# Kmatsuo57/cell-image-analysis

Hardware: AMD Instinct MI355X
Metric: cells/sec screened (CAE fwd + recon-MSE + SVM score), 64x64 (higher is better)
Workload: dtype f32 (results in the fp32 error class; the contractions run as split 16-bit products on the matrix pipe, fp32 accumulate: conv1..conv6 as 2 fp16 terms x 3 products with exact power-of-two scales from each cell's own data, the PCA GEMM as 3 bf16 terms x 6 products, conv7's 32 -> 16 channel contraction; 1 GPU; BASELINE.json configs[2]: screening inference, 1000000 synthetic 64x64 crops on one GPU, resident in HBM, CAE fwd + recon MSE/MAE + RobustScaler + PCA(100) + 2x OCSVM score on device; cells_per_gpu=1000000, global_cells=1000000, chunk_cells=65536, detector_train_cells=5000, weights=random init (Glorot, non-trivial BN), seed 42, parallelism=dp1

## Files before the change

cell-image-analysis_amd/csrc/conv12_fused.hip:

```cpp
#include "kernel_setup.hpp"
#include "split16.hpp"

#include <cmath>
#include <cstdlib>
#include <cstring>
#include <type_traits>
#include <vector>

namespace cs {

namespace {

constexpr int NTHR = 512;
constexpr int V_BYTES = 36 * 2048;
constexpr int RING_SLOTS = 10;
constexpr int RING_ROWF = 34 * 32 + 8;
static_assert((4 * RING_ROWF) % 64 == 32 && RING_ROWF % 2 == 0, "ring pitch");
constexpr int RING_BYTES = RING_SLOTS * RING_ROWF * 4;
constexpr int E2_BYTES = 8 * 2048;
constexpr int INP_STRIDE = 72;
constexpr int INP_BYTES = 67 * INP_STRIDE * 4;
constexpr int OFF_RING = V_BYTES;
constexpr int OFF_E2 = OFF_RING + RING_BYTES;
constexpr int OFF_INP = OFF_E2 + E2_BYTES;
// ... 116 lines not shown
    if (tid < 384) ((float*)(smem + OFF_B1))[tid] = w1frag[tid];
    if (tid < 32) {
        const float sc = ep1[32 + tid];
        ((f32x4*)(smem + OFF_EP1))[tid] = f32x4{ep1[tid], sc, ep1[64 + tid], sc >= 0.0f ? 1.0f : -1.0f};
    }
    if (tid >= 64 && tid < 128) {
        const int c = tid - 64;
        const float sc = ep2[64 + c];
        ((f32x4*)(smem + OFF_EP2))[c] = f32x4{ep2[c], sc, ep2[128 + c], sc >= 0.0f ? 1.0f : -1.0f};
    }
    if constexpr (C1H) {
        for (int i = tid; i < (2 * 2 * 64 * 16) / 4; i += NTHR) ((unsigned int*)(smem + OFF_B1X))[i] = w1x3[i];
    }
    {
        const int srow = tid >> 4, sc16 = tid & 15;
        const float* src = x + (size_t)blockIdx.x * 4096 + srow * 64 + 4 * sc16;
        float* dst = inp + (srow + 1) * INP_STRIDE + 4 + 4 * sc16;
        f32x4 c0 = *(const f32x4*)src, c1 = *(const f32x4*)(src + 32 * 64);
        c12_sanitize(c0);
        c12_sanitize(c1);
        *(f32x4*)dst = c0;
        *(f32x4*)(dst + 32 * INP_STRIDE) = c1;
        if constexpr (C2H) {
            const unsigned int mx = f16x2_rowmax(f16x2_absmax8(c0, c1));
            if ((lane & 15) == 0) atomicMax((unsigned int*)(smem + OFF_XMAX), mx);
        }
    }
    __syncthreads();
    float vscale = 1.0f, vunscale = 1.0f, xscale = 1.0f, xunscale = 1.0f;
    auto set_scale = [&]() {
        const float xm = __builtin_bit_cast(float, *(const unsigned int*)(smem + OFF_XMAX));
        if constexpr (C1H) {
            int Ex = (int)((__builtin_bit_cast(unsigned int, xm) >> 23) & 0xffu);
            Ex = Ex < 40 ? 40 : (Ex > 254 ? 254 : Ex);
            Ex = __builtin_amdgcn_readfirstlane(Ex);
            xscale = __builtin_bit_cast(float, (unsigned int)(268 - Ex) << 23);
            xunscale = __builtin_bit_cast(float, (unsigned int)(Ex - 14) << 23) * inv_sw1;
        }
        const float vb = 100.0f * fmaf(p1a, xm, p1b);
        int E = (int)((__builtin_bit_cast(unsigned int, vb) >> 23) & 0xffu);
        E = E < 40 ? 40 : (E > 254 ? 254 : E);
        E = __builtin_amdgcn_readfirstlane(E);
        vscale = __builtin_bit_cast(float, (unsigned int)(268 - E) << 23);
        vunscale = __builtin_bit_cast(float, (unsigned int)(E - 14) << 23) * inv_sw;
    };
    if constexpr (C2H) set_scale();
    auto records_in_place = [&](int t) {
        float* p0 = inp + ((t >> 4) + 1) * INP_STRIDE + 4 + 4 * (t & 15);
// ... 152 lines not shown
                const float* const rcol = ring + (4 * tx) * 32 + 2 * p;
                auto p2_body = [&](auto lo_c) {
                    constexpr bool LO = decltype(lo_c)::value;
                    f32x2 t[3][6];
                    {
                        const float* rrow[5];
    #pragma unroll
                        for (int m = 0; m < 5; ++m) {
                            const unsigned int sm = (unsigned int)(rbase + m);
                            const unsigned int slot = min(sm, sm - (unsigned int)RING_SLOTS);
                            rrow[m] = rcol + slot * RING_ROWF;
                        }
                        f32x2 d[6][5];
    #pragma unroll
                        for (int j = 0; j < 6; ++j)
    #pragma unroll
                            for (int m = 0; m < 5; ++m) d[j][m] = lds_read_b64(rrow[m] + j * 32);
                        if (g == 3 && has_next) {
                            float* dst = inp + ((t2 >> 4) + 1) * INP_STRIDE + 4 + 4 * (t2 & 15);
                            c12_sanitize(stg0);
                            c12_sanitize(stg1);
                            *(f32x4*)dst = stg0;
                            *(f32x4*)(dst + 32 * INP_STRIDE) = stg1;
                            const unsigned int mx = f16x2_rowmax(f16x2_absmax8(stg0, stg1));
                            if ((l2 & 15) == 0) atomicMax((unsigned int*)(smem + OFF_XMAX), mx);
                        }
    #pragma unroll
                        for (int j = 0; j < 6; ++j) {
                            f32x2 o[3];
                            bt6_half<LO>(d[j], o);
    #pragma unroll
                            for (int rr = 0; rr < 3; ++rr) t[rr][j] = o[rr];
                        }
                    }
                    const int sx = (tile >> 1) & 7;
                    char* const vhi = smem + (3 * h) * (6 * 2048) + (tile * 8 + ((p >> 2) ^ sx)) * 16 + (p & 3) * 4;
                    char* const vlo = smem + (3 * h) * (6 * 2048) + (tile * 8 + ((4 + (p >> 2)) ^ sx)) * 16 + (p & 3) * 4;
    #pragma unroll
                    for (int rr = 0; rr < 3; ++rr) {
                        f32x2 o[6];
                        bt6_pair(t[rr], o);
                        unsigned int ph[6], pl[6];
                        f16x2_split6_pairs(o, ph, pl);
    #pragma unroll
                        for (int c = 0; c < 6; ++c) {
                            *(unsigned int*)(vhi + (rr * 6 + c) * 2048) = ph[c];
                            *(unsigned int*)(vlo + (rr * 6 + c) * 2048) = pl[c];
                        }
// ... 316 lines not shown
```

cell-image-analysis_amd/csrc/conv45_h2.hip:

```cpp
#include "kernel_setup.hpp"
#include "split16.hpp"

#include <cstring>

namespace cs {

namespace {

constexpr int G = 8;
constexpr int CH = 32;
constexpr int WP = G + 2;
constexpr int PXB = 64;
constexpr int ROWB = WP * PXB + 32;
constexpr int PLANE = WP * ROWB;
constexpr int WG_PER_CU = 2;

constexpr int C5_OUT = 64;

constexpr int H2_OFF_MAX = 2 * PLANE;
constexpr int H2_LDS_BYTES = 2 * PLANE + 16;

__device__ __forceinline__ void h2_split_store(char* dst, const f32x4& x, float S)
{
    f16x4 hi;
// ... 15 lines not shown
    const int th = wave >> 1;
    const int li = lane & 15, kq = lane >> 4;

    f16x8 B[9][2];
#pragma unroll
    for (int t = 0; t < 9; ++t)
#pragma unroll
        for (int p = 0; p < 2; ++p) B[t][p] = wfrag[((slice * 9 + t) * 2 + p) * 64 + lane];
    const int co = slice * 16 + li;
    const float bias = ep[co], bns = ep[CH + co], bnt = ep[2 * CH + co];

    for (int i = tid; i < H2_LDS_BYTES / 16; i += 256) *(f32x4*)(smem + i * 16) = f32x4{0.0f, 0.0f, 0.0f, 0.0f};

    long cell = blockIdx.x;
    if (cell >= n_cells) return;
    f32x4 stg[2];
#pragma unroll
    for (int k = 0; k < 2; ++k) stg[k] = *(const f32x4*)(in + (size_t)cell * (G * G * CH) + (tid + 256 * k) * 4);
    __syncthreads();
    {
        unsigned int mx = 0;
        f16x2_absmax4(stg[0], mx);
        f16x2_absmax4(stg[1], mx);
        mx = f16x2_rowmax(mx);
        if (li == 0) atomicMax(&mxw[0], mx);
    }
    __syncthreads();
    float S, invS;
    f16x2_scale(mxw[0], S, invS);

    int woff[2];
#pragma unroll
    for (int k = 0; k < 2; ++k) {
        const int idx = tid + 256 * k, px = idx >> 3, c4 = idx & 7;
        woff[k] = ((px >> 3) + 1) * ROWB + ((px & 7) + 1) * PXB + c4 * 8;
    }
    const int abase = (4 * th + (li >> 3)) * ROWB + (li & 7) * PXB + kq * 16;

    for (int it = 0; cell < n_cells; cell += gridDim.x, ++it) {
        const float unscale = invS * inv_sw;
#pragma unroll
        for (int k = 0; k < 2; ++k) h2_split_store(smem + woff[k], stg[k], S);
        __syncthreads();
        if (tid == 0) mxw[it & 1] = 0;
        const long ncell = cell + gridDim.x;
        if (ncell < n_cells) {
#pragma unroll
            for (int k = 0; k < 2; ++k) stg[k] = *(const f32x4*)(in + (size_t)ncell * (G * G * CH) + (tid + 256 * k) * 4);
// ... 7 lines not shown
#pragma unroll
            for (int t = 0; t < 2; ++t) {
                const char* a = smem + abase + toff + t * (2 * ROWB);
                const f16x8 a1 = *(const f16x8*)a;
                const f16x8 a2 = *(const f16x8*)(a + PLANE);
                lo[t] = __builtin_amdgcn_mfma_f32_16x16x32_f16(a1, B[tap][1], lo[t], 0, 0, 0);
                hi[t] = __builtin_amdgcn_mfma_f32_16x16x32_f16(a1, B[tap][0], hi[t], 0, 0, 0);
                lo[t] = __builtin_amdgcn_mfma_f32_16x16x32_f16(a2, B[tap][0], lo[t], 0, 0, 0);
            }
        }
#pragma unroll
        for (int t = 0; t < 2; ++t) {
            float* o = out + ((size_t)cell * (G * G) + 16 * (2 * th + t) + 4 * kq) * CH + co;
#pragma unroll
            for (int r = 0; r < 4; ++r) {
                const float v = fmaxf(fmaf(hi[t][r] + lo[t][r], unscale, bias), 0.0f);
                o[r * CH] = fmaf(v, bns, bnt);
            }
        }
        if (ncell < n_cells) {
            unsigned int mx = 0;
            f16x2_absmax4(stg[0], mx);
            f16x2_absmax4(stg[1], mx);
            mx = f16x2_rowmax(mx);
            if (li == 0) atomicMax(&mxw[(it + 1) & 1], mx);
        }
        __syncthreads();
        f16x2_scale(mxw[(it + 1) & 1], S, invS);
    }
}

__global__ __launch_bounds__(512, 2) void conv5_h2_kernel(const float* __restrict__ in, const f16x8* __restrict__ wfrag,
                                                          const float* __restrict__ ep, float* __restrict__ out, long n_cells, float inv_sw)
{
    extern __shared__ __attribute__((aligned(16))) char smem[];
    unsigned int* const mxw = (unsigned int*)(smem + H2_OFF_MAX);
    const int tid = threadIdx.x;
    const int lane = tid & 63;
    const int wave = __builtin_amdgcn_readfirstlane(tid >> 6);
    const int ph = wave >> 1, pa = ph >> 1, pb = ph & 1;
    const int sp = wave & 1;
    const int li = lane & 15, kq = lane >> 4;

    f16x8 B[4][2][2];
#pragma unroll
    for (int t = 0; t < 4; ++t)
#pragma unroll
        for (int k = 0; k < 2; ++k)
#pragma unroll
            for (int p = 0; p < 2; ++p) B[t][k][p] = wfrag[(((wave * 4 + t) * 2 + k) * 2 + p) * 64 + lane];
    float bias[2], bns[2], bnt[2];
#pragma unroll
    for (int k = 0; k < 2; ++k) {
        const int co = (2 * sp + k) * 16 + li;
        bias[k] = ep[co]; bns[k] = ep[C5_OUT + co]; bnt[k] = ep[2 * C5_OUT + co];
    }

    for (int i = tid; i < H2_LDS_BYTES / 16; i += 512) *(f32x4*)(smem + i * 16) = f32x4{0.0f, 0.0f, 0.0f, 0.0f};

    long cell = blockIdx.x;
    if (cell >= n_cells) return;
    f32x4 stg = *(const f32x4*)(in + (size_t)cell * (G * G * CH) + tid * 4);
    __syncthreads();
    {
        unsigned int mx = 0;
        f16x2_absmax4(stg, mx);
        mx = f16x2_rowmax(mx);
        if (li == 0) atomicMax(&mxw[0], mx);
    }
    __syncthreads();
    float S, invS;
    f16x2_scale(mxw[0], S, invS);
    const int woff = ((tid >> 6) + 1) * ROWB + (((tid >> 3) & 7) + 1) * PXB + (tid & 7) * 8;
    const int abase = ((li >> 3) + pa) * ROWB + ((li & 7) + pb) * PXB + kq * 16;

    for (int it = 0; cell < n_cells; cell += gridDim.x, ++it) {
        const float unscale = invS * inv_sw;
        h2_split_store(smem + woff, stg, S);
        __syncthreads();
        if (tid == 0) mxw[it & 1] = 0;
        const long ncell = cell + gridDim.x;
        if (ncell < n_cells) stg = *(const f32x4*)(in + (size_t)ncell * (G * G * CH) + tid * 4);

        float* obase = out + (((size_t)cell * (2 * G) + pa) * (2 * G) + pb) * C5_OUT + (2 * sp) * 16 + li;
#pragma unroll
        for (int t = 0; t < 4; ++t) {
            f32x4 ah[2] = {{0.0f, 0.0f, 0.0f, 0.0f}, {0.0f, 0.0f, 0.0f, 0.0f}};
            f32x4 al[2] = {{0.0f, 0.0f, 0.0f, 0.0f}, {0.0f, 0.0f, 0.0f, 0.0f}};
#pragma unroll
            for (int tap = 0; tap < 4; ++tap) {
                const char* a = smem + abase + t * (2 * ROWB) + (tap >> 1) * ROWB + (tap & 1) * PXB;
                const f16x8 a1 = *(const f16x8*)a;
                const f16x8 a2 = *(const f16x8*)(a + PLANE);
#pragma unroll
                for (int k = 0; k < 2; ++k) {
                    al[k] = __builtin_amdgcn_mfma_f32_16x16x32_f16(a1, B[tap][k][1], al[k], 0, 0, 0);
                    ah[k] = __builtin_amdgcn_mfma_f32_16x16x32_f16(a1, B[tap][k][0], ah[k], 0, 0, 0);
                    al[k] = __builtin_amdgcn_mfma_f32_16x16x32_f16(a2, B[tap][k][0], al[k], 0, 0, 0);
                }
            }
#pragma unroll
            for (int r = 0; r < 4; ++r) {
                const int i = 4 * kq + r, ys = 2 * t + (i >> 3), xs = i & 7;
                float* o = obase + ((size_t)(2 * ys) * (2 * G) + 2 * xs) * C5_OUT;
#pragma unroll
                for (int k = 0; k < 2; ++k) {
                    const float v = fmaxf(fmaf(ah[k][r] + al[k][r], unscale, bias[k]), 0.0f);
                    o[16 * k] = fmaf(v, bns[k], bnt[k]);
                }
            }
        }
        if (ncell < n_cells) {
            unsigned int mx = 0;
            f16x2_absmax4(stg, mx);
            mx = f16x2_rowmax(mx);
            if (li == 0) atomicMax(&mxw[(it + 1) & 1], mx);
        }
        __syncthreads();
        f16x2_scale(mxw[(it + 1) & 1], S, invS);
    }
}

constexpr int F45_OFF_A = 2 * PLANE;
constexpr int F45_OFF_W4 = 4 * PLANE;
constexpr int F45_W4_BYTES = 2 * 9 * 2 * 64 * 16;
constexpr int F45_OFF_MAX = F45_OFF_W4 + F45_W4_BYTES;
constexpr int F45_LDS_BYTES = F45_OFF_MAX + 16;
static_assert(2 * F45_LDS_BYTES <= 160 * 1024, "two workgroups per CU");

__global__ __launch_bounds__(512, 2) void conv45_h2_kernel(const float* __restrict__ in , const f16x8* __restrict__ w4frag,
                                                           const float* __restrict__ ep4, float inv_sw4, const f16x8* __restrict__ w5frag,
                                                           const float* __restrict__ ep5, float inv_sw5, float* __restrict__ out ,
                                                           long n_cells)
{
    extern __shared__ __attribute__((aligned(16))) char smem[];
    unsigned int* const mxw = (unsigned int*)(smem + F45_OFF_MAX);
    const int tid = threadIdx.x;
    const int lane = tid & 63;
    const int wave = __builtin_amdgcn_readfirstlane(tid >> 6);
// ... 8 lines not shown
#pragma unroll
        for (int k = 0; k < 2; ++k)
#pragma unroll
            for (int p = 0; p < 2; ++p) B[t][k][p] = w5frag[(((wave * 4 + t) * 2 + k) * 2 + p) * 64 + lane];
    float bias[2], bns[2], bnt[2];
#pragma unroll
    for (int k = 0; k < 2; ++k) {
        const int co = (2 * sp + k) * 16 + li;
        bias[k] = ep5[co]; bns[k] = ep5[C5_OUT + co]; bnt[k] = ep5[2 * C5_OUT + co];
    }
    const int co4 = slice4 * 16 + li;
    const float bias4 = ep4[co4], bns4 = ep4[CH + co4], bnt4 = ep4[2 * CH + co4];

    for (int i = tid; i < F45_LDS_BYTES / 16; i += 512) *(f32x4*)(smem + i * 16) = f32x4{0.0f, 0.0f, 0.0f, 0.0f};
    __syncthreads();
    for (int i = tid; i < F45_W4_BYTES / 16; i += 512) *(f16x8*)(smem + F45_OFF_W4 + i * 16) = w4frag[i];

    long cell = blockIdx.x;
    if (cell >= n_cells) return;
    f32x4 stg = *(const f32x4*)(in + (size_t)cell * (G * G * CH) + tid * 4);
    {
        unsigned int mx = 0;
        f16x2_absmax4(stg, mx);
        mx = f16x2_rowmax(mx);
        if (li == 0) atomicMax(&mxw[0], mx);
    }
    __syncthreads();
    float S3, invS3;
    f16x2_scale(mxw[0], S3, invS3);
    const int woff = ((tid >> 6) + 1) * ROWB + (((tid >> 3) & 7) + 1) * PXB + (tid & 7) * 8;
    const int abase4 = (2 * tile4 + (li >> 3)) * ROWB + (li & 7) * PXB + kq * 16;
    const char* const w4l = smem + F45_OFF_W4 + (size_t)slice4 * 9 * 2 * 64 * 16 + lane * 16;
    const int abase5 = F45_OFF_A + ((li >> 3) + pa) * ROWB + ((li & 7) + pb) * PXB + kq * 16;

    for (int it = 0; cell < n_cells; cell += gridDim.x, ++it) {
        h2_split_store(smem + woff, stg, S3);
        __syncthreads();
        if (tid == 0) mxw[it & 1] = 0;
        const long ncell = cell + gridDim.x;
        if (ncell < n_cells) stg = *(const f32x4*)(in + (size_t)ncell * (G * G * CH) + tid * 4);

        f32x4 a4v;
        {
            f32x4 hi = {0.0f, 0.0f, 0.0f, 0.0f}, lo = {0.0f, 0.0f, 0.0f, 0.0f};
#pragma unroll
            for (int tap = 0; tap < 9; ++tap) {
                const char* a = smem + abase4 + (tap / 3) * ROWB + (tap % 3) * PXB;
                const f16x8 a1 = *(const f16x8*)a;
                const f16x8 a2 = *(const f16x8*)(a + PLANE);
                const f16x8 bh = *(const f16x8*)(w4l + (tap * 2 + 0) * 1024), bl = *(const f16x8*)(w4l + (tap * 2 + 1) * 1024);
                lo = __builtin_amdgcn_mfma_f32_16x16x32_f16(a1, bl, lo, 0, 0, 0);
                hi = __builtin_amdgcn_mfma_f32_16x16x32_f16(a1, bh, hi, 0, 0, 0);
                lo = __builtin_amdgcn_mfma_f32_16x16x32_f16(a2, bh, lo, 0, 0, 0);
            }
            const float us4 = invS3 * inv_sw4;
            float am = 0.0f;
#pragma unroll
            for (int r = 0; r < 4; ++r) {
                const float v = fmaxf(fmaf(hi[r] + lo[r], us4, bias4), 0.0f);
                a4v[r] = fmaf(v, bns4, bnt4);
                am = fmaxf(am, fabsf(a4v[r]));
            }
            const unsigned int m = f16x2_rowmax(__builtin_bit_cast(unsigned int, am));
            if (li == 0) atomicMax(&mxw[2 + (it & 1)], m);
        }
        __syncthreads();
        float S4, invS4;
        f16x2_scale(mxw[2 + (it & 1)], S4, invS4);
        {
#pragma unroll
            for (int r = 0; r < 4; ++r) {
                const int p = 16 * tile4 + 4 * kq + r;
                char* d = smem + F45_OFF_A + ((p >> 3) + 1) * ROWB + ((p & 7) + 1) * PXB + co4 * 2;
                const float v = a4v[r] * S4;
                const _Float16 h = (_Float16)v;
                *(_Float16*)d = h;
                *(_Float16*)(d + PLANE) = (_Float16)(v - (float)h);
            }
        }
        __syncthreads();
        if (tid == 0) mxw[2 + (it & 1)] = 0;

        const float unscale = invS4 * inv_sw5;
        float* obase = out + (((size_t)cell * (2 * G) + pa) * (2 * G) + pb) * C5_OUT + (2 * sp) * 16 + li;
#pragma unroll
        for (int t = 0; t < 4; ++t) {
            f32x4 ah[2] = {{0.0f, 0.0f, 0.0f, 0.0f}, {0.0f, 0.0f, 0.0f, 0.0f}};
// ... 4 lines not shown
                const f16x8 a1 = *(const f16x8*)a;
                const f16x8 a2 = *(const f16x8*)(a + PLANE);
#pragma unroll
                for (int k = 0; k < 2; ++k) {
                    al[k] = __builtin_amdgcn_mfma_f32_16x16x32_f16(a1, B[tap][k][1], al[k], 0, 0, 0);
                    ah[k] = __builtin_amdgcn_mfma_f32_16x16x32_f16(a1, B[tap][k][0], ah[k], 0, 0, 0);
                    al[k] = __builtin_amdgcn_mfma_f32_16x16x32_f16(a2, B[tap][k][0], al[k], 0, 0, 0);
                }
            }
#pragma unroll
            for (int r = 0; r < 4; ++r) {
                const int i = 4 * kq + r, ys = 2 * t + (i >> 3), xs = i & 7;
                float* o = obase + ((size_t)(2 * ys) * (2 * G) + 2 * xs) * C5_OUT;
#pragma unroll
                for (int k = 0; k < 2; ++k) {
                    const float v = fmaxf(fmaf(ah[k][r] + al[k][r], unscale, bias[k]), 0.0f);
                    o[16 * k] = fmaf(v, bns[k], bnt[k]);
                }
            }
        }
        if (ncell < n_cells) {
            unsigned int mx = 0;
            f16x2_absmax4(stg, mx);
            mx = f16x2_rowmax(mx);
            if (li == 0) atomicMax(&mxw[(it + 1) & 1], mx);
        }
        __syncthreads();
        f16x2_scale(mxw[(it + 1) & 1], S3, invS3);
    }
}

}

size_t pack_conv4_f16x2(const float* hwio, uint16_t* dst, float* inv_sw)
{
    const size_t n = (size_t)2 * 9 * 2 * 64 * 8;
    if (!dst) return n;
    const float S = f16x2_weight_scale(hwio, (size_t)9 * CH * CH);
    if (inv_sw) *inv_sw = 1.0f / S;
    for (int s = 0; s < 2; ++s)
        for (int t = 0; t < 9; ++t)
            for (int l = 0; l < 64; ++l)
                for (int j = 0; j < 8; ++j) {
                    const int li = l & 15, kq = l >> 4;
                    uint16_t pl[2];
                    f16x2_split(hwio[((size_t)t * CH + 8 * kq + j) * CH + 16 * s + li], S, pl[0], pl[1]);
                    for (int p = 0; p < 2; ++p) dst[((((size_t)s * 9 + t) * 2 + p) * 64 + l) * 8 + j] = pl[p];
                }
// ... 58 lines not shown
```

cell-image-analysis_amd/csrc/conv_wino_cs.hip:

```cpp
#include "kernel_setup.hpp"
#include "split16.hpp"

#include <cmath>
#include <cstdlib>
#include <cstring>
#include <vector>

namespace cs {

namespace {

template <int H_, int W_, int CIN_, int COUT_>
struct WinoCfg {
    static constexpr int H = H_, W = W_, CIN = CIN_, COUT = COUT_;
    static constexpr int TW = W / 2;
    static constexpr int TR = 16 / TW;
    static constexpr int SR = 2 * TR;
    static constexpr int R = SR + 2, WP = W + 2;
    static constexpr int PS = CIN + 4;
    static constexpr int STRIP = R * WP * PS * 4;
    static constexpr int NQ = CIN / 16, NS = COUT / 16, KS = CIN / 4;
    static constexpr int NB = 4 * NS * KS;
    static constexpr int XCH = 4 * NS * 2 * 64 * 16;
    static constexpr int LDS = 2 * STRIP + XCH;
// ... 240 lines not shown

    const long total = n_cells * C::NGRP;
    const long first = blockIdx.x;
    if (first >= total) return;
    const int spx = tid / C::C4, sc4 = tid % C::C4;
    const int goff = spx * C::CIN + sc4 * 4, loff = (spx + 1) * C::PS + sc4 * 4;
    auto cell_ptr = [&](long cell) { return in + (size_t)cell * C::H * C::W * C::CIN; };
    auto st_prep = [&](int y0, int r, f32x4 v, unsigned int& mx) {
        const int sy = y0 - 1 + r;
        if (sy < 0 || sy >= C::H) v = f32x4{0.0f, 0.0f, 0.0f, 0.0f};
        f16x2_absmax4(v, mx);
        return v;
    };
    for (int i = tid; i < W3H::LDS / 16; i += 256) ((f32x4*)smem)[i] = f32x4{0.0f, 0.0f, 0.0f, 0.0f};
    __syncthreads();
    float S, invS;
    {
        unsigned int mx = 0;
#pragma unroll
        for (int r = 0; r < C::R; ++r) {
            const f32x4 v = st_prep((int)(first % C::NGRP) * C::SR, r, wn_load<C>(cell_ptr(first / C::NGRP), (int)(first % C::NGRP) * C::SR, r, goff), mx);
            *(f32x4*)((float*)smem + r * W3X::ROWP + loff) = v;
        }
        mx = f16x2_rowmax(mx);
        if (li == 0) atomicMax(&mxw[0], mx);
        __syncthreads();
        f16x2_scale<2>(mxw[0], S, invS);
        __syncthreads();
        if (tid == 0) mxw[0] = 0;
    }

    f32x4 stg[C::NLD];
    int buf = 0;
    int k = 0;
    for (long item = first; item < total; item += gridDim.x, ++k) {
        const long cell = item / C::NGRP;
        const int grp = (int)(item % C::NGRP);
        const long nitem = item + gridDim.x;
        const bool has_next = nitem < total;
        const float* strip = (const float*)(smem + buf * W3X::STRIP);
        float* nstrip = (float*)(smem + (buf ^ 1) * W3X::STRIP);
        unsigned int* const mword = mxw + ((k + 1) & 1);
        const float unscale = invS * inv_sw;
        if (has_next) {
#pragma unroll
            for (int j = 0; j < C::NLD; ++j) stg[j] = wn_load<C>(cell_ptr(nitem / C::NGRP), (int)(nitem % C::NGRP) * C::SR, j, goff);
        }
        const float* da_p = strip + poff + ca * C::PS;
// ... 30 lines not shown
                    acc[s][r] = d;
                }
            }
        }
#pragma unroll
        for (int s = 0; s < C::NS; ++s) {
            f32x4 s0, s1;
#pragma unroll
            for (int r = 0; r < 4; ++r) {
                s0[r] = (acc[s][0][r] + acc[s][1][r]) + acc[s][2][r];
                s1[r] = (acc[s][1][r] - acc[s][2][r]) - acc[s][3][r];
            }
            float* x = xch + ((size_t)((wc * C::NS + s) * 2) * 64 + lane) * 4;
            *(f32x4*)x = s0;
            *(f32x4*)(x + 64 * 4) = s1;
        }
        if (has_next) {
            unsigned int mx = 0;
#pragma unroll
            for (int j = 0; j < C::NLD; ++j) {
                stg[j] = st_prep((int)(nitem % C::NGRP) * C::SR, j, stg[j], mx);
                *(f32x4*)(nstrip + j * W3X::ROWP + loff) = stg[j];
            }
            mx = f16x2_rowmax(mx);
            if (li == 0) atomicMax(mword, mx);
        }
        __syncthreads();
        if (has_next) f16x2_scale<2>(*mword, S, invS);
        f32x4 t0[4], t1[4];
#pragma unroll
        for (int c = 0; c < 4; ++c) {
            const float* x = xch + ((size_t)((c * C::NS + fs) * 2) * 64 + lane) * 4;
            t0[c] = *(const f32x4*)x;
            t1[c] = *(const f32x4*)(x + 64 * 4);
        }
        const f32x4 y00 = (t0[0] + t0[1]) + t0[2], y01 = (t0[1] - t0[2]) - t0[3];
        const f32x4 y10 = (t1[0] + t1[1]) + t1[2], y11 = (t1[1] - t1[2]) - t1[3];
        auto post = [&](float v) { v = fmaxf(fmaf(v, unscale, bias), 0.0f); return fmaf(v, bns, bnt); };
#pragma unroll
        for (int rr = 0; rr < C::FR; ++rr) {
            const float a = rbase ? y00[2 + rr] : y00[rr], b = rbase ? y01[2 + rr] : y01[rr];
            const float c2 = rbase ? y10[2 + rr] : y10[rr], d = rbase ? y11[2 + rr] : y11[rr];
            const float mx = fmaxf(fmaxf(a, b), fmaxf(c2, d)), mn = fminf(fminf(a, b), fminf(c2, d));
            const float res = post(bns >= 0.0f ? mx : mn);
            const int t = 4 * kq + rbase + rr;
            const int ty = grp * C::TR + t / C::TW, tx = t % C::TW;
            out[(((size_t)cell * (C::H / 2) + ty) * (C::W / 2) + tx) * C::COUT + co] = res;
        }
// ... 284 lines not shown
```

cell-image-analysis_amd/csrc/conv_wino_up.hip:

```cpp
#include "kernel_setup.hpp"
#include "split16.hpp"

#include <type_traits>

#include <cmath>
#include <cstdlib>
#include <cstring>

namespace cs {

namespace {

template <int HS_, int WS_, int CIN_, int COUT_>
struct WUCfg {
    static constexpr int HS = HS_, WS = WS_, CIN = CIN_, COUT = COUT_;
    static constexpr int HO = 2 * HS, WO = 2 * WS;
    static constexpr int TW = WS / 2;
    static constexpr int SR = 2 * (16 / TW);
    static constexpr int R = SR + 2, WP = WS + 2;
    static constexpr int PS = CIN + 4;
    static constexpr int STRIP = R * WP * PS * 4;
    static constexpr int LDS = 2 * STRIP;
    static constexpr int NGRP = HS / SR;
    static constexpr int NQ = CIN / 16, KS = CIN / 4;
// ... 454 lines not shown
#pragma unroll
            for (int p = 0; p < 2; ++p) B[t][k][p] = wfrag[(((wave * 4 + t) * 2 + k) * 2 + p) * 64 + lane];
    const int co = wsl * 16 + li;
    const int cosw = co ^ ((kq & 1) << 4);
    const float bias = ep[co], bns = ep[C::COUT + co], bnt = ep[2 * C::COUT + co];
    const float b7 = b7p[0];

    const long first = blockIdx.x;
    if (first >= n_cells) return;
    const int se = tid & (C::EPR - 1), rsub = tid / C::EPR;
    const int spx = se / C::C4, sc4 = se & (C::C4 - 1);
    const int goff = spx * C::CIN + sc4 * 4;
    const int loffb = (spx + 1) * F67H::PXB + sc4 * 8;
    auto cell_ptr = [&](long cell) { return in + (size_t)cell * C::HS * C::WS * C::CIN; };
    for (int i = tid; i < F67H::LDS / 16; i += C::THREADS) ((f32x4*)smem)[i] = f32x4{0.0f, 0.0f, 0.0f, 0.0f};
    __syncthreads();
    wl[(tid >> 5) * F67H::WP + (tid & 31)] = weff[tid];
    float unscale;
    {
        f32x4 stg[C::NLD];
        unsigned int mx = 0;
#pragma unroll
        for (int j = 0; j < C::NLD; ++j) stg[j] = h2_prep(0, j, rsub, wu_load<C>(cell_ptr(first), 0, j, rsub, goff), mx);
        mx = f16x2_rowmax(mx);
        if (li == 0) atomicMax(&mxw[0], mx);
        __syncthreads();
        float S, invS;
        f16x2_scale(mxw[0], S, invS);
        unscale = invS * inv_sw;
#pragma unroll
        for (int j = 0; j < C::NLD; ++j) h2_store(smem, j, rsub, loffb, stg[j], S);
    }
    __syncthreads();
    if (tid == 0) mxw[0] = 0;
    const char* abase = smem + (pa * 18 + li + pb) * F67H::PXB + kq * 16;

    int strip_no = 0;
    for (long cell = first; cell < n_cells; cell += gridDim.x) {
        const float* xc = x + (size_t)cell * 64 * 64;
        float s2 = 0.0f, s1 = 0.0f;
#pragma unroll 1
        for (int grp = 0; grp < C::NGRP; ++grp) {
            const long ncell = grp < C::NGRP - 1 ? cell : cell + gridDim.x;
            const int ngrp = grp < C::NGRP - 1 ? grp + 1 : 0;
            const bool has_next = ncell < n_cells;
            ++strip_no;
            unsigned int* const mword = mxw + (strip_no & 1);

            if constexpr (DIAG) dt = cycle_stamp();
            f32x4 stg[C::NLD];
            if (has_next) {
#pragma unroll
                for (int j = 0; j < C::NLD; ++j) stg[j] = wu_load<C>(cell_ptr(ncell), ngrp * C::SR, j, rsub, goff);
            }
            float xv[2];
#pragma unroll
            for (int h = 0; h < 2; ++h) {
                const int k = wave + 8 * h, o = 2 * (8 * grp + (k >> 1)) - 1 + (k & 1);
                xv[h] = xc[(o < 0 ? 0 : o) * 64 + lane];
            }
            float xtail = 0.0f;
            if (grp == C::NGRP - 1 && wave == 0) xtail = xc[63 * 64 + lane];

            if constexpr (DIAG) { const unsigned long long t = cycle_stamp(); dg[0] += t - dt; dt = t; }
            f32x4 ah[4], al[4];
#pragma unroll
            for (int t = 0; t < 4; ++t) ah[t] = al[t] = f32x4{0.0f, 0.0f, 0.0f, 0.0f};
            auto rd = [&](int f, f16x8 (&a)[2]) {
                const int sr = f >> 2, rx = (f >> 1) & 1, k = f & 1;
                const char* p = abase + sr * F67H::ROWB + rx * F67H::PXB + k * 64;
                a[0] = *(const f16x8*)p;
                a[1] = *(const f16x8*)(p + F67H::PLB);
            };
            auto mac3 = [&](const f16x8 (&a)[2], const f16x8 (&b)[2], f32x4& dh, f32x4& dl) {
                dl = __builtin_amdgcn_mfma_f32_16x16x32_f16(a[0], b[1], dl, 0, 0, 0);
                dh = __builtin_amdgcn_mfma_f32_16x16x32_f16(a[0], b[0], dh, 0, 0, 0);
                dl = __builtin_amdgcn_mfma_f32_16x16x32_f16(a[1], b[0], dl, 0, 0, 0);
            };
            {
                f16x8 a[2];
                rd(0, a);
                __builtin_amdgcn_sched_group_barrier(0x100, 2, 0);
#pragma unroll
                for (int f = 0; f < 20; ++f) {
                    const int sr = f >> 2, rx = (f >> 1) & 1, k = f & 1;
                    f16x8 an[2] = {a[0], a[1]};
                    if (f + 1 < 20) rd(f + 1, an);
                    if (sr < 4) mac3(a, B[rx][k], ah[sr], al[sr]);
                    if (sr > 0) mac3(a, B[2 + rx][k], ah[sr - 1], al[sr - 1]);
                    a[0] = an[0]; a[1] = an[1];
                    __builtin_amdgcn_sched_group_barrier(0x100, 2, 0);
                    if (sr > 0 && sr < 4) __builtin_amdgcn_sched_group_barrier(0x008, 6, 0);
                    else __builtin_amdgcn_sched_group_barrier(0x008, 3, 0);
                }
            }
            if constexpr (DIAG) {
                asm volatile("" ::"v"(ah[0][0]), "v"(al[3][3]));
                const unsigned long long t = cycle_stamp(); dg[1] += t - dt; dt = t;
            }
#pragma unroll
            for (int t = 0; t < 4; ++t)
#pragma unroll
                for (int r = 0; r < 4; ++r) {
                    const float v = fmaxf(fmaf(ah[t][r] + al[t][r], unscale, bias), 0.0f);
                    a6s[((2 * t + pa) * 32 + 2 * (4 * kq + r) + pb) * F67H::PA + cosw] = fmaf(v, bns, bnt);
                }
            if (has_next) {
                unsigned int mx = 0;
#pragma unroll
                for (int j = 0; j < C::NLD; ++j) stg[j] = h2_prep(ngrp * C::SR, j, rsub, stg[j], mx);
                mx = f16x2_rowmax(mx);
                if (li == 0) atomicMax(mword, mx);
            }
            __syncthreads();
            if constexpr (DIAG) { const unsigned long long t = cycle_stamp(); dg[2] += t - dt; dt = t; }
            {
                const int wrow = 4 * ((li >> 3) | (((li >> 2) & 1) << 1)) + (li & 3);
                float wc[8];
                *(f32x4*)&wc[0] = *(const f32x4*)(wl + wrow * F67H::WP + 4 * kq);
                *(f32x4*)&wc[4] = *(const f32x4*)(wl + wrow * F67H::WP + 4 * kq + 16);
                const int pix = 4 * (li & 3) + (li >> 2), sw = ((li >> 1) & 1) << 4;
                const float* ap = a6s + (wave * 32 + pix) * F67H::PA + 4 * kq;
                const f32x4 a00 = *(const f32x4*)(ap + sw), a01 = *(const f32x4*)(ap + (sw ^ 16));
                const f32x4 a10 = *(const f32x4*)(ap + 16 * F67H::PA + sw), a11 = *(const f32x4*)(ap + 16 * F67H::PA + (sw ^ 16));
                f32x4 t0 = f32x4{0.0f, 0.0f, 0.0f, 0.0f}, t1 = t0;
#pragma unroll
                for (int s = 0; s < 4; ++s) {
                    t0 = __builtin_amdgcn_mfma_f32_16x16x4f32(wc[s], a00[s], t0, 0, 0, 0);
                    t1 = __builtin_amdgcn_mfma_f32_16x16x4f32(wc[s], a10[s], t1, 0, 0, 0);
                }
#pragma unroll
                for (int s = 0; s < 4; ++s) {
                    t0 = __builtin_amdgcn_mfma_f32_16x16x4f32(wc[4 + s], a01[s], t0, 0, 0, 0);
                    t1 = __builtin_amdgcn_mfma_f32_16x16x4f32(wc[4 + s], a11[s], t1, 0, 0, 0);
                }
                const int rblk = kq == 0 ? 0 : (kq == 1 ? 3 : (kq == 2 ? 1 : 2));
                float* tw = tb + ((((8 * grp + wave) & (F67::TSLOTS - 1)) * 16) + 4 * rblk) * F67H::TW + pix + 1 - (kq >> 1);
#pragma unroll
                for (int r = 0; r < 4; ++r) { tw[r * F67H::TW] = t0[r]; tw[r * F67H::TW + 16] = t1[r]; }
            }
            if (has_next) {
                float S, invS;
                f16x2_scale(*mword, S, invS);
                unscale = invS * inv_sw;
#pragma unroll
                for (int j = 0; j < C::NLD; ++j) h2_store(smem, j, rsub, loffb, stg[j], S);
            }
            __syncthreads();
            if (tid == 0) *mword = 0;
            if constexpr (DIAG) { const unsigned long long t = cycle_stamp(); dg[3] += t - dt; dt = t; }
            const int px = lane & 1, xh = lane >> 1;
#pragma unroll
            for (int h = 0; h < 2; ++h) {
                const int k = wave + 8 * h;
                const int y = 8 * grp + (k >> 1), e = k & 1;
                if (2 * y - 1 + e < 0) continue;
                const int nb = (e ? px : 3 - px) * 4;
                const float* ra = tb + ((((y - 1) & (F67::TSLOTS - 1)) * 16) + nb) * F67H::TW + xh;
                const float* rb = tb + (((y & (F67::TSLOTS - 1)) * 16) + nb) * F67H::TW + xh;
                float ta0 = ra[0], ta1 = ra[F67H::TW + 1];
                const float tb0 = rb[2 * F67H::TW], tb1 = rb[3 * F67H::TW + 1];
                if (y == 0) { ta0 = 0.0f; ta1 = 0.0f; }
                const float v = ((ta0 + ta1) + (tb0 + tb1)) + b7;
                const float rr = f67_sigmoid(v);
                const float d = xv[h] - rr;
                s2 = fmaf(d, d, s2);
                s1 += fabsf(d);
            }
            if (grp == C::NGRP - 1 && wave == 0) {
                const int nb = (3 - px) * 4;
                const float* ra = tb + (((31 & (F67::TSLOTS - 1)) * 16) + nb) * F67H::TW + xh;
                const float v = (ra[0] + ra[F67H::TW + 1]) + b7;
                const float rr = f67_sigmoid(v);
                const float d = xtail - rr;
                s2 = fmaf(d, d, s2);
                s1 += fabsf(d);
            }
            if constexpr (DIAG) {
                asm volatile("" ::"v"(s2), "v"(s1));
                const unsigned long long t = cycle_stamp(); dg[4] += t - dt; dt = t;
            }
        }
#pragma unroll
        for (int off = 32; off > 0; off >>= 1) {
            s2 += __shfl_down(s2, off, 64);
            s1 += __shfl_down(s1, off, 64);
        }
        if (lane == 0) {
            errpart[((size_t)cell * F67::NPARTS + wave) * 2 + 0] = s2;
            errpart[((size_t)cell * F67::NPARTS + wave) * 2 + 1] = s1;
        }
    }
    if constexpr (DIAG) {
        if (lane == 0) {
#pragma unroll
            for (int k = 0; k < 5; ++k) diag[((size_t)blockIdx.x * 8 + wave) * 5 + k] = dg[k];
        }
    }
}

template <class C>
size_t pack_frags(const float* hwio, float* dst)
{
    const size_t total = (size_t)8 * C::NB * 64;
    if (!dst) return total;
    static const double G[3][2] = {{1, 0}, {1, 1}, {0, 1}};
    for (int ph = 0; ph < 4; ++ph)
        for (int half = 0; half < 2; ++half)
            for (int k = 0; k < C::NSW; ++k)
                for (int xi = 0; xi < 9; ++xi)
                    for (int kk = 0; kk < C::KS; ++kk)
                        for (int lane = 0; lane < 64; ++lane) {
                            const int a = ph >> 1, b = ph & 1, li = lane & 15, kq = lane >> 4, q = kk >> 2, j = kk & 3;
                            const int ci = 16 * q + 4 * kq + j, co = 16 * (half * C::NSW + k) + li, r = xi / 3, c = xi % 3;
                            double u = 0.0;
// ... 121 lines not shown
```

cell-image-analysis_amd/csrc/split16.hpp:

```cpp
#pragma once
#include "common.hpp"

#include <cmath>
#include <cstring>

namespace cs {

typedef _Float16 f16x8 __attribute__((ext_vector_type(8)));
typedef _Float16 f16x4 __attribute__((ext_vector_type(4)));
typedef _Float16 f16x2 __attribute__((ext_vector_type(2)));
typedef unsigned int u32x4 __attribute__((ext_vector_type(4)));
typedef unsigned int u32x2 __attribute__((ext_vector_type(2)));
typedef float f32x2 __attribute__((ext_vector_type(2)));

__device__ __forceinline__ unsigned int f16x2_rowmax(unsigned int m)
{
    unsigned int o;
    o = (unsigned int)__builtin_amdgcn_update_dpp(0, (int)m, 0xB1, 0xF, 0xF, true);  m = m > o ? m : o;
    o = (unsigned int)__builtin_amdgcn_update_dpp(0, (int)m, 0x4E, 0xF, 0xF, true);  m = m > o ? m : o;
    o = (unsigned int)__builtin_amdgcn_update_dpp(0, (int)m, 0x124, 0xF, 0xF, true); m = m > o ? m : o;
    o = (unsigned int)__builtin_amdgcn_update_dpp(0, (int)m, 0x128, 0xF, 0xF, true); m = m > o ? m : o;
    return m;
}

template <int BIAS = 0>
__device__ __forceinline__ void f16x2_scale(unsigned int mbits, float& S, float& invS)
{
    int E = (int)((mbits >> 23) & 0xffu) + BIAS;
    E = E < 40 ? 40 : (E > 254 ? 254 : E);
    S = __builtin_bit_cast(float, (unsigned int)(268 - E) << 23);
    invS = __builtin_bit_cast(float, (unsigned int)(E - 14) << 23);
}

__device__ __forceinline__ float f16x2_absmax4(const f32x4& v)
{
    const float a = v[0], b = v[1], c = v[2], d = v[3];
    return fmaxf(fmaxf(fabsf(a), fabsf(b)), fmaxf(fabsf(c), fabsf(d)));
}
__device__ __forceinline__ void f16x2_absmax4(const f32x4& v, unsigned int& mx)
{
    const unsigned int u = __builtin_bit_cast(unsigned int, f16x2_absmax4(v));
    mx = mx > u ? mx : u;
}
__device__ __forceinline__ unsigned int f16x2_absmax8(const f32x4& a, const f32x4& b)
{
// ... 134 lines not shown
```

Measured before the change: 5.683 million cells/s.

## Pipeline conv6/7 up kernel: defer recon-error gather, fuse hi/lo accumulators, wave-level max

Adds a helper that reduces the per-row absmax across the four 16-lane rows with readlane and issues one LDS atomicMax per wave instead of four, and applies it in every conv kernel. In the conv6/conv7 upsampling kernel, the sigmoid/MSE gather for the previous strip is deferred by one iteration and interleaved with the MFMA loop. The next strip's h2_prep and scale-and-store work is moved inside the MFMA and conv7 phases with explicit sched_group_barrier interleaving. The hi and lo MFMA accumulators are merged into one, and next-cell loads are made unconditional by clamping to the current cell. This cuts accumulator registers, adds, atomics and serialized phases. In exchange it changes the summation order slightly and makes the scheduling more fragile.

```diff
diff --git a/cell-image-analysis_amd/csrc/conv12_fused.hip b/cell-image-analysis_amd/csrc/conv12_fused.hip
--- a/cell-image-analysis_amd/csrc/conv12_fused.hip
+++ b/cell-image-analysis_amd/csrc/conv12_fused.hip
@@ -162,8 +162,7 @@
         *(f32x4*)dst = c0;
         *(f32x4*)(dst + 32 * INP_STRIDE) = c1;
         if constexpr (C2H) {
-            const unsigned int mx = f16x2_rowmax(f16x2_absmax8(c0, c1));
-            if ((lane & 15) == 0) atomicMax((unsigned int*)(smem + OFF_XMAX), mx);
+            f16x2_wave_atomic_max((unsigned int*)(smem + OFF_XMAX), f16x2_rowmax(f16x2_absmax8(c0, c1)), lane);
         }
     }
     __syncthreads();
@@ -362,8 +361,7 @@
                             c12_sanitize(stg1);
                             *(f32x4*)dst = stg0;
                             *(f32x4*)(dst + 32 * INP_STRIDE) = stg1;
-                            const unsigned int mx = f16x2_rowmax(f16x2_absmax8(stg0, stg1));
-                            if ((l2 & 15) == 0) atomicMax((unsigned int*)(smem + OFF_XMAX), mx);
+                            f16x2_wave_atomic_max((unsigned int*)(smem + OFF_XMAX), f16x2_rowmax(f16x2_absmax8(stg0, stg1)), l2);
                         }
     #pragma unroll
                         for (int j = 0; j < 6; ++j) {
diff --git a/cell-image-analysis_amd/csrc/conv45_h2.hip b/cell-image-analysis_amd/csrc/conv45_h2.hip
--- a/cell-image-analysis_amd/csrc/conv45_h2.hip
+++ b/cell-image-analysis_amd/csrc/conv45_h2.hip
@@ -61,8 +61,7 @@
         unsigned int mx = 0;
         f16x2_absmax4(stg[0], mx);
         f16x2_absmax4(stg[1], mx);
-        mx = f16x2_rowmax(mx);
-        if (li == 0) atomicMax(&mxw[0], mx);
+        f16x2_wave_atomic_max(&mxw[0], f16x2_rowmax(mx), lane);
     }
     __syncthreads();
     float S, invS;
@@ -116,8 +115,7 @@
             unsigned int mx = 0;
             f16x2_absmax4(stg[0], mx);
             f16x2_absmax4(stg[1], mx);
-            mx = f16x2_rowmax(mx);
-            if (li == 0) atomicMax(&mxw[(it + 1) & 1], mx);
+            f16x2_wave_atomic_max(&mxw[(it + 1) & 1], f16x2_rowmax(mx), lane);
         }
         __syncthreads();
         f16x2_scale(mxw[(it + 1) & 1], S, invS);
@@ -159,8 +157,7 @@
     {
         unsigned int mx = 0;
         f16x2_absmax4(stg, mx);
-        mx = f16x2_rowmax(mx);
-        if (li == 0) atomicMax(&mxw[0], mx);
+        f16x2_wave_atomic_max(&mxw[0], f16x2_rowmax(mx), lane);
     }
     __syncthreads();
     float S, invS;
@@ -207,8 +204,7 @@
         if (ncell < n_cells) {
             unsigned int mx = 0;
             f16x2_absmax4(stg, mx);
-            mx = f16x2_rowmax(mx);
-            if (li == 0) atomicMax(&mxw[(it + 1) & 1], mx);
+            f16x2_wave_atomic_max(&mxw[(it + 1) & 1], f16x2_rowmax(mx), lane);
         }
         __syncthreads();
         f16x2_scale(mxw[(it + 1) & 1], S, invS);
@@ -263,8 +259,7 @@
     {
         unsigned int mx = 0;
         f16x2_absmax4(stg, mx);
-        mx = f16x2_rowmax(mx);
-        if (li == 0) atomicMax(&mxw[0], mx);
+        f16x2_wave_atomic_max(&mxw[0], f16x2_rowmax(mx), lane);
     }
     __syncthreads();
     float S3, invS3;
@@ -302,8 +297,7 @@
                 a4v[r] = fmaf(v, bns4, bnt4);
                 am = fmaxf(am, fabsf(a4v[r]));
             }
-            const unsigned int m = f16x2_rowmax(__builtin_bit_cast(unsigned int, am));
-            if (li == 0) atomicMax(&mxw[2 + (it & 1)], m);
+            f16x2_wave_atomic_max(&mxw[2 + (it & 1)], f16x2_rowmax(__builtin_bit_cast(unsigned int, am)), lane);
         }
         __syncthreads();
         float S4, invS4;
@@ -354,8 +348,7 @@
         if (ncell < n_cells) {
             unsigned int mx = 0;
             f16x2_absmax4(stg, mx);
-            mx = f16x2_rowmax(mx);
-            if (li == 0) atomicMax(&mxw[(it + 1) & 1], mx);
+            f16x2_wave_atomic_max(&mxw[(it + 1) & 1], f16x2_rowmax(mx), lane);
         }
         __syncthreads();
         f16x2_scale(mxw[(it + 1) & 1], S3, invS3);
diff --git a/cell-image-analysis_amd/csrc/conv_wino_cs.hip b/cell-image-analysis_amd/csrc/conv_wino_cs.hip
--- a/cell-image-analysis_amd/csrc/conv_wino_cs.hip
+++ b/cell-image-analysis_amd/csrc/conv_wino_cs.hip
@@ -286,8 +286,7 @@
             const f32x4 v = st_prep((int)(first % C::NGRP) * C::SR, r, wn_load<C>(cell_ptr(first / C::NGRP), (int)(first % C::NGRP) * C::SR, r, goff), mx);
             *(f32x4*)((float*)smem + r * W3X::ROWP + loff) = v;
         }
-        mx = f16x2_rowmax(mx);
-        if (li == 0) atomicMax(&mxw[0], mx);
+        f16x2_wave_atomic_max(&mxw[0], f16x2_rowmax(mx), lane);
         __syncthreads();
         f16x2_scale<2>(mxw[0], S, invS);
         __syncthreads();
@@ -364,8 +363,7 @@
                 stg[j] = st_prep((int)(nitem % C::NGRP) * C::SR, j, stg[j], mx);
                 *(f32x4*)(nstrip + j * W3X::ROWP + loff) = stg[j];
             }
-            mx = f16x2_rowmax(mx);
-            if (li == 0) atomicMax(mword, mx);
+            f16x2_wave_atomic_max(mword, f16x2_rowmax(mx), lane);
         }
         __syncthreads();
         if (has_next) f16x2_scale<2>(*mword, S, invS);
diff --git a/cell-image-analysis_amd/csrc/conv_wino_up.hip b/cell-image-analysis_amd/csrc/conv_wino_up.hip
--- a/cell-image-analysis_amd/csrc/conv_wino_up.hip
+++ b/cell-image-analysis_amd/csrc/conv_wino_up.hip
@@ -500,8 +500,7 @@
         unsigned int mx = 0;
 #pragma unroll
         for (int j = 0; j < C::NLD; ++j) stg[j] = h2_prep(0, j, rsub, wu_load<C>(cell_ptr(first), 0, j, rsub, goff), mx);
-        mx = f16x2_rowmax(mx);
-        if (li == 0) atomicMax(&mxw[0], mx);
+        f16x2_wave_atomic_max(&mxw[0], f16x2_rowmax(mx), lane);
         __syncthreads();
         float S, invS;
         f16x2_scale(mxw[0], S, invS);
@@ -512,83 +511,144 @@
     __syncthreads();
     if (tid == 0) mxw[0] = 0;
     const char* abase = smem + (pa * 18 + li + pb) * F67H::PXB + kq * 16;
+    int a6b[4][2];
+#pragma unroll
+    for (int t = 0; t < 4; ++t)
+#pragma unroll
+        for (int h = 0; h < 2; ++h) {
+            a6b[t][h] = F67H::STRIP + (((2 * t + pa) * 32 + 2 * (4 * kq + 2 * h) + pb) * F67H::PA + cosw) * 4;
+            asm volatile("" : "+v"(a6b[t][h]));
+        }
+
+    const int px = lane & 1, xh = lane >> 1;
+    float s2 = 0.0f, s1 = 0.0f;
+    auto gather = [&](int g, bool live, const float (&xq)[2]) {
+#pragma unroll
+        for (int h = 0; h < 2; ++h) {
+            const int k = wave + 8 * h;
+            const int y = 8 * g + (k >> 1), e = k & 1;
+            const int nb = (e ? px : 3 - px) * 4;
+            const float* ra = tb + ((((y - 1) & (F67::TSLOTS - 1)) * 16) + nb) * F67H::TW + xh;
+            const float* rb = tb + (((y & (F67::TSLOTS - 1)) * 16) + nb) * F67H::TW + xh;
+            float ta0 = ra[0], ta1 = ra[F67H::TW + 1];
+            const float tb0 = rb[2 * F67H::TW], tb1 = rb[3 * F67H::TW + 1];
+            unsigned int m0 = y == 0 ? 0u : ~0u;
+            unsigned int md = (live && 2 * y - 1 + e >= 0) ? ~0u : 0u;
+            asm("" : "+v"(m0), "+v"(md));
+            const float sa = __builtin_bit_cast(float, __builtin_bit_cast(unsigned int, ta0 + ta1) & m0);
+            const float v = (sa + (tb0 + tb1)) + b7;
+            const float rr = f67_sigmoid(v);
+            const float d = __builtin_bit_cast(float, __builtin_bit_cast(unsigned int, xq[h] - rr) & md);
+            s2 = fmaf(d, d, s2);
+            s1 += fabsf(d);
+        }
+    };
+    auto finish_cell = [&](long c, float xt) {
+        if (wave == 0) {
+            const int nb = (3 - px) * 4;
+            const float* ra = tb + (((31 & (F67::TSLOTS - 1)) * 16) + nb) * F67H::TW + xh;
+            const float v = (ra[0] + ra[F67H::TW + 1]) + b7;
+            const float rr = f67_sigmoid(v);
+            const float d = xt - rr;
+            s2 = fmaf(d, d, s2);
+            s1 += fabsf(d);
+        }
+#pragma unroll
+        for (int off = 32; off > 0; off >>= 1) {
+            s2 += __shfl_down(s2, off, 64);
+            s1 += __shfl_down(s1, off, 64);
+        }
+        if (lane == 0) {
+            errpart[((size_t)c * F67::NPARTS + wave) * 2 + 0] = s2;
+            errpart[((size_t)c * F67::NPARTS + wave) * 2 + 1] = s1;
+        }
+        s2 = 0.0f;
+        s1 = 0.0f;
+    };
 
     int strip_no = 0;
+    float xvp[2] = {0.0f, 0.0f}, xtail = 0.0f;
+    bool live = false;
+    long pcell = first;
+    constexpr int FB = 13;
     for (long cell = first; cell < n_cells; cell += gridDim.x) {
         const float* xc = x + (size_t)cell * 64 * 64;
-        float s2 = 0.0f, s1 = 0.0f;
 #pragma unroll 1
         for (int grp = 0; grp < C::NGRP; ++grp) {
             const long ncell = grp < C::NGRP - 1 ? cell : cell + gridDim.x;
             const int ngrp = grp < C::NGRP - 1 ? grp + 1 : 0;
-            const bool has_next = ncell < n_cells;
+            const long lcell = ncell < n_cells ? ncell : cell;
             ++strip_no;
             unsigned int* const mword = mxw + (strip_no & 1);
 
             if constexpr (DIAG) dt = cycle_stamp();
             f32x4 stg[C::NLD];
-            if (has_next) {
-#pragma unroll
-                for (int j = 0; j < C::NLD; ++j) stg[j] = wu_load<C>(cell_ptr(ncell), ngrp * C::SR, j, rsub, goff);
-            }
+#pragma unroll
+            for (int j = 0; j < C::NLD; ++j) stg[j] = wu_load<C>(cell_ptr(lcell), ngrp * C::SR, j, rsub, goff);
             float xv[2];
 #pragma unroll
             for (int h = 0; h < 2; ++h) {
                 const int k = wave + 8 * h, o = 2 * (8 * grp + (k >> 1)) - 1 + (k & 1);
                 xv[h] = xc[(o < 0 ? 0 : o) * 64 + lane];
             }
-            float xtail = 0.0f;
             if (grp == C::NGRP - 1 && wave == 0) xtail = xc[63 * 64 + lane];
 
             if constexpr (DIAG) { const unsigned long long t = cycle_stamp(); dg[0] += t - dt; dt = t; }
-            f32x4 ah[4], al[4];
-#pragma unroll
-            for (int t = 0; t < 4; ++t) ah[t] = al[t] = f32x4{0.0f, 0.0f, 0.0f, 0.0f};
+            f32x4 acc[4];
+#pragma unroll
+            for (int t = 0; t < 4; ++t) acc[t] = f32x4{0.0f, 0.0f, 0.0f, 0.0f};
             auto rd = [&](int f, f16x8 (&a)[2]) {
                 const int sr = f >> 2, rx = (f >> 1) & 1, k = f & 1;
                 const char* p = abase + sr * F67H::ROWB + rx * F67H::PXB + k * 64;
                 a[0] = *(const f16x8*)p;
                 a[1] = *(const f16x8*)(p + F67H::PLB);
             };
-            auto mac3 = [&](const f16x8 (&a)[2], const f16x8 (&b)[2], f32x4& dh, f32x4& dl) {
-                dl = __builtin_amdgcn_mfma_f32_16x16x32_f16(a[0], b[1], dl, 0, 0, 0);
-                dh = __builtin_amdgcn_mfma_f32_16x16x32_f16(a[0], b[0], dh, 0, 0, 0);
-                dl = __builtin_amdgcn_mfma_f32_16x16x32_f16(a[1], b[0], dl, 0, 0, 0);
+            auto mac3 = [&](const f16x8 (&a)[2], const f16x8 (&b)[2], f32x4& d) {
+                d = __builtin_amdgcn_mfma_f32_16x16x32_f16(a[0], b[1], d, 0, 0, 0);
+                d = __builtin_amdgcn_mfma_f32_16x16x32_f16(a[1], b[0], d, 0, 0, 0);
+                d = __builtin_amdgcn_mfma_f32_16x16x32_f16(a[0], b[0], d, 0, 0, 0);
             };
             {
+                gather((grp + C::NGRP - 1) & (C::NGRP - 1), live, xvp);
                 f16x8 a[2];
                 rd(0, a);
                 __builtin_amdgcn_sched_group_barrier(0x100, 2, 0);
+                unsigned int mx = 0;
 #pragma unroll
                 for (int f = 0; f < 20; ++f) {
                     const int sr = f >> 2, rx = (f >> 1) & 1, k = f & 1;
+                    if (f == FB) {
+                        asm volatile("" : "+v"(s2), "+v"(s1));
+                        __builtin_amdgcn_sched_barrier(0);
+#pragma unroll
+                        for (int j = 0; j < C::NLD; ++j) stg[j] = h2_prep(ngrp * C::SR, j, rsub, stg[j], mx);
+                    }
                     f16x8 an[2] = {a[0], a[1]};
                     if (f + 1 < 20) rd(f + 1, an);
-                    if (sr < 4) mac3(a, B[rx][k], ah[sr], al[sr]);
-                    if (sr > 0) mac3(a, B[2 + rx][k], ah[sr - 1], al[sr - 1]);
+                    if (sr < 4) mac3(a, B[rx][k], acc[sr]);
+                    if (sr > 0) mac3(a, B[2 + rx][k], acc[sr - 1]);
                     a[0] = an[0]; a[1] = an[1];
-                    __builtin_amdgcn_sched_group_barrier(0x100, 2, 0);
-                    if (sr > 0 && sr < 4) __builtin_amdgcn_sched_group_barrier(0x008, 6, 0);
-                    else __builtin_amdgcn_sched_group_barrier(0x008, 3, 0);
-                }
-            }
-            if constexpr (DIAG) {
-                asm volatile("" ::"v"(ah[0][0]), "v"(al[3][3]));
-                const unsigned long long t = cycle_stamp(); dg[1] += t - dt; dt = t;
-            }
-#pragma unroll
-            for (int t = 0; t < 4; ++t)
-#pragma unroll
-                for (int r = 0; r < 4; ++r) {
-                    const float v = fmaxf(fmaf(ah[t][r] + al[t][r], unscale, bias), 0.0f);
-                    a6s[((2 * t + pa) * 32 + 2 * (4 * kq + r) + pb) * F67H::PA + cosw] = fmaf(v, bns, bnt);
-                }
-            if (has_next) {
-                unsigned int mx = 0;
-#pragma unroll
-                for (int j = 0; j < C::NLD; ++j) stg[j] = h2_prep(ngrp * C::SR, j, rsub, stg[j], mx);
-                mx = f16x2_rowmax(mx);
-                if (li == 0) atomicMax(mword, mx);
+                    if (f < 8) __builtin_amdgcn_sched_group_barrier(0x100, 3, 0);
+                    else __builtin_amdgcn_sched_group_barrier(0x100, 2, 0);
+#pragma unroll
+                    for (int m = 0; m < ((sr > 0 && sr < 4) ? 6 : 3); ++m) {
+                        __builtin_amdgcn_sched_group_barrier(0x008, 1, 0);
+                        if (sr == 4) __builtin_amdgcn_sched_group_barrier(0x402, 2, 0);
+                        else __builtin_amdgcn_sched_group_barrier(0x402, 1, 0);
+                    }
+                }
+                if constexpr (DIAG) {
+                    asm volatile("" ::"v"(acc[0][0]), "v"(acc[3][3]), "v"(s2), "v"(s1), "v"(mx));
+                    const unsigned long long t = cycle_stamp(); dg[1] += t - dt; dt = t;
+                }
+#pragma unroll
+                for (int t = 0; t < 4; ++t)
+#pragma unroll
+                    for (int r = 0; r < 4; ++r) {
+                        const float v = fmaxf(fmaf(acc[t][r], unscale, bias), 0.0f);
+                        *(float*)(smem + a6b[t][r >> 1] + (r & 1) * (2 * F67H::PA * 4)) = fmaf(v, bns, bnt);
+                    }
+                f16x2_wave_atomic_max(mword, f16x2_rowmax(mx), lane);
             }
             __syncthreads();
             if constexpr (DIAG) { const unsigned long long t = cycle_stamp(); dg[2] += t - dt; dt = t; }
@@ -601,6 +661,9 @@
                 const float* ap = a6s + (wave * 32 + pix) * F67H::PA + 4 * kq;
                 const f32x4 a00 = *(const f32x4*)(ap + sw), a01 = *(const f32x4*)(ap + (sw ^ 16));
                 const f32x4 a10 = *(const f32x4*)(ap + 16 * F67H::PA + sw), a11 = *(const f32x4*)(ap + 16 * F67H::PA + (sw ^ 16));
+                float S, invS;
+                f16x2_scale(*mword, S, invS);
+                unscale = invS * inv_sw;
                 f32x4 t0 = f32x4{0.0f, 0.0f, 0.0f, 0.0f}, t1 = t0;
 #pragma unroll
                 for (int s = 0; s < 4; ++s) {
@@ -612,63 +675,35 @@
                     t0 = __builtin_amdgcn_mfma_f32_16x16x4f32(wc[4 + s], a01[s], t0, 0, 0, 0);
                     t1 = __builtin_amdgcn_mfma_f32_16x16x4f32(wc[4 + s], a11[s], t1, 0, 0, 0);
                 }
+#pragma unroll
+                for (int j = 0; j < C::NLD; ++j) h2_store(smem, j, rsub, loffb, stg[j], S);
                 const int rblk = kq == 0 ? 0 : (kq == 1 ? 3 : (kq == 2 ? 1 : 2));
                 float* tw = tb + ((((8 * grp + wave) & (F67::TSLOTS - 1)) * 16) + 4 * rblk) * F67H::TW + pix + 1 - (kq >> 1);
 #pragma unroll
                 for (int r = 0; r < 4; ++r) { tw[r * F67H::TW] = t0[r]; tw[r * F67H::TW + 16] = t1[r]; }
-            }
-            if (has_next) {
-                float S, invS;
-                f16x2_scale(*mword, S, invS);
-                unscale = invS * inv_sw;
-#pragma unroll
-                for (int j = 0; j < C::NLD; ++j) h2_store(smem, j, rsub, loffb, stg[j], S);
+                __builtin_amdgcn_sched_group_barrier(0x100, 7, 0);
+#pragma unroll
+                for (int m = 0; m < 16; ++m) {
+                    __builtin_amdgcn_sched_group_barrier(0x008, 1, 0);
+                    __builtin_amdgcn_sched_group_barrier(0x402, 4, 0);
+                    __builtin_amdgcn_sched_group_barrier(0x200, 1, 0);
+                }
             }
             __syncthreads();
             if (tid == 0) *mword = 0;
             if constexpr (DIAG) { const unsigned long long t = cycle_stamp(); dg[3] += t - dt; dt = t; }
-            const int px = lane & 1, xh = lane >> 1;
-#pragma unroll
-            for (int h = 0; h < 2; ++h) {
-                const int k = wave + 8 * h;
-                const int y = 8 * grp + (k >> 1), e = k & 1;
-                if (2 * y - 1 + e < 0) continue;
-                const int nb = (e ? px : 3 - px) * 4;
-                const float* ra = tb + ((((y - 1) & (F67::TSLOTS - 1)) * 16) + nb) * F67H::TW + xh;
-                const float* rb = tb + (((y & (F67::TSLOTS - 1)) * 16) + nb) * F67H::TW + xh;
-                float ta0 = ra[0], ta1 = ra[F67H::TW + 1];
-                const float tb0 = rb[2 * F67H::TW], tb1 = rb[3 * F67H::TW + 1];
-                if (y == 0) { ta0 = 0.0f; ta1 = 0.0f; }
-                const float v = ((ta0 + ta1) + (tb0 + tb1)) + b7;
-                const float rr = f67_sigmoid(v);
-                const float d = xv[h] - rr;
-                s2 = fmaf(d, d, s2);
-                s1 += fabsf(d);
-            }
-            if (grp == C::NGRP - 1 && wave == 0) {
-                const int nb = (3 - px) * 4;
-                const float* ra = tb + (((31 & (F67::TSLOTS - 1)) * 16) + nb) * F67H::TW + xh;
-                const float v = (ra[0] + ra[F67H::TW + 1]) + b7;
-                const float rr = f67_sigmoid(v);
-                const float d = xtail - rr;
-                s2 = fmaf(d, d, s2);
-                s1 += fabsf(d);
-            }
+            if (grp == 0 && live) finish_cell(pcell, xtail);
+            xvp[0] = xv[0]; xvp[1] = xv[1];
+            live = true;
+            pcell = cell;
             if constexpr (DIAG) {
-                asm volatile("" ::"v"(s2), "v"(s1));
+                asm volatile("" ::"v"(xvp[0]), "v"(xvp[1]));
                 const unsigned long long t = cycle_stamp(); dg[4] += t - dt; dt = t;
             }
         }
-#pragma unroll
-        for (int off = 32; off > 0; off >>= 1) {
-            s2 += __shfl_down(s2, off, 64);
-            s1 += __shfl_down(s1, off, 64);
-        }
-        if (lane == 0) {
-            errpart[((size_t)cell * F67::NPARTS + wave) * 2 + 0] = s2;
-            errpart[((size_t)cell * F67::NPARTS + wave) * 2 + 1] = s1;
-        }
     }
+    gather(C::NGRP - 1, true, xvp);
+    finish_cell(pcell, xtail);
     if constexpr (DIAG) {
         if (lane == 0) {
 #pragma unroll
diff --git a/cell-image-analysis_amd/csrc/split16.hpp b/cell-image-analysis_amd/csrc/split16.hpp
--- a/cell-image-analysis_amd/csrc/split16.hpp
+++ b/cell-image-analysis_amd/csrc/split16.hpp
@@ -21,6 +21,15 @@
     o = (unsigned int)__builtin_amdgcn_update_dpp(0, (int)m, 0x124, 0xF, 0xF, true); m = m > o ? m : o;
     o = (unsigned int)__builtin_amdgcn_update_dpp(0, (int)m, 0x128, 0xF, 0xF, true); m = m > o ? m : o;
     return m;
+}
+
+__device__ __forceinline__ void f16x2_wave_atomic_max(unsigned int* word, unsigned int rowmax, int lane)
+{
+    const unsigned int a = (unsigned int)__builtin_amdgcn_readlane((int)rowmax, 0), b = (unsigned int)__builtin_amdgcn_readlane((int)rowmax, 16);
+    const unsigned int c = (unsigned int)__builtin_amdgcn_readlane((int)rowmax, 32), d = (unsigned int)__builtin_amdgcn_readlane((int)rowmax, 48);
+    const unsigned int ab = a > b ? a : b, cd = c > d ? c : d;
+    const unsigned int m = ab > cd ? ab : cd;
+    if (lane == 0) atomicMax(word, m);
 }
 
 template <int BIAS = 0>
```

Result: no change. 5.685 million cells/s, median of 2 (+0.0%).
